# frankaging/Multimodal-Transformer

Hardware: AMD Instinct MI355X
Metric: windows/sec fwd+bwd (higher is better)
Workload: dtype bf16; 1 GPU; SFT encoder stack T=500 d_model=128 heads=8 N=6 d_ff=128, 32 sequences/GPU; fwd + MSE loss + bwd (input, weight, LayerNorm grads); global_batch=32, seq_len=500, d_model=128, heads=8, layers=6, d_ff=128, parallelism=dp1, dropout=train mode, p=0.10 at the reference's four encoder sites, in-kernel generator, lengths=full

## Files before the change

multimodal_transformer_amd/csrc/api.hip:

```cpp
#include <hip/hip_runtime.h>
#include <stdarg.h>
#include <stdio.h>
#include <string.h>
#include <math.h>
#include <stdlib.h>
#include <mutex>
#include <type_traits>
#include <unordered_set>

#include "../../include/mmt_hip.h"
#include "common.h"
#include "rowgemm.h"
#include "attn_mask.h"
#include "attn.h"
#include "attn_bwd_pair.h"
#include "attn_probs.h"
#ifdef MMT_ABLATIONS
#include "attn_bwd_pair_diag.h"
#include "attn_fwd_diag.h"
#endif
#include "misc_kernels.h"
#include "scan_common.h"
#include "scan.h"
#include "mfn_scan.h"
#include "scan_units.h"
#include "scan256.h"
#include "scan_cluster.h"
#include "scan_stack_plan.h"
#include "scan_stack.h"
#include "scan_fb_plan.h"
#include "scan_fb.h"
#include "convpool.h"
#include "convk.h"
#include "glue.h"
#include "local_attn.h"
#include "ar_combine.h"

static thread_local char g_err[512] = "";
static int fail(int code, const char* fmt, ...) {
    va_list ap; va_start(ap, fmt); vsnprintf(g_err, sizeof(g_err), fmt, ap); va_end(ap);
    return code;
}
#define HIP_TRY(expr) do { hipError_t e_ = (expr); if (e_ != hipSuccess) \
    return fail(MMT_EHIP, "%s failed: %s (%s:%d)", #expr, hipGetErrorString(e_), __FILE__, __LINE__); } while (0)

static int ensure_dynamic_lds(const void* kernel) {
// ... 224 lines not shown
        W.slab_stride = set_bytes / sizeof(float);
        for (int l = 1; l < D.N; ++l) c.take<char>(set_bytes);
    }
    for (int l = 0; l < D.N; ++l) { W.lw[l].maskQ = nullptr; W.lw[l].maskK = nullptr; }
    if (train) {
        const size_t lw = attn_mask_layer_words(D.B * D.h, D.nt);
        uint16_t* mq = c.take<uint16_t>(lw * (size_t)(D.N > 0 ? D.N : 1));
        uint16_t* mk = c.take<uint16_t>(lw * (size_t)(D.N > 0 ? D.N : 1));
        for (int l = 0; l < D.N; ++l) { W.lw[l].maskQ = mq ? mq + lw * l : nullptr; W.lw[l].maskK = mk ? mk + lw * l : nullptr; }
    }
    W.bytes = c.off;
}

template <int EPI, bool LN, bool WIDE = false, bool DEVSEED = false>
static int launch_rowgemm(const RowGemmParams& p, hipStream_t st, int site = S_OTHER) {
    if (EPI == EPI_LNBWD && !WIDE && p.no_gs) return launch_rowgemm<EPI_LNBWD, false, true>(p, st, site);
    if (EPI == EPI_PLAIN && !DEVSEED && p.seedword) return launch_rowgemm<EPI_PLAIN, LN, WIDE, true>(p, st, site);
    if (!WIDE && (p.no_gs || p.kchunk)) return fail(MMT_EINVAL, "K-chunked staging / single-tile column sums exist for the LayerNorm-backward kernel only");
    const size_t lds = rowgemm_lds_bytes(EPI, LN, p.KP, p.NP, p.kchunk, p.no_gs != 0);
    if (lds > 160 * 1024) return fail(MMT_EUNSUPPORTED, "row GEMM tile needs %zu B of LDS (K=%d, N=%d)", lds, p.K, p.N);
    if (WIDE && p.kchunk && (!p.a_bf16 || (p.kchunk & (p.kchunk - 1)) || p.kchunk < 64 || p.A_out))
        return fail(MMT_EINVAL, "K-chunked staging needs a bf16 A matrix, a power-of-two chunk >= 64 and no A copy");
    ProfScope prof(site, st);
    return launch("rowgemm_kernel", rowgemm_kernel<EPI, LN, WIDE, DEVSEED>, dim3((p.M + MMT_ROWS - 1) / MMT_ROWS), dim3(MMT_RTHREADS), lds, st, p);
}

static int launch_rowgemm_fixed(void (*kernel)(RowGemmParams), const RowGemmParams& p, size_t lds, hipStream_t st, int site, const char* name) {
    ProfScope prof(site, st);
    return launch(name, kernel, dim3((p.M + MMT_ROWS - 1) / MMT_ROWS), dim3(MMT_RTHREADS), lds, st, p);
}

static int chain_extra_kp(const RowChain3&) { return 0; }
static int chain_extra_kp(const RowChain4& ch) { return ch.d.KP; }

template <typename CH>
static int launch_rowchain(void (*kernel)(CH), CH& ch, bool lnbwd, int site, const char* name, hipStream_t st, int lnb_np = 0, int shape = 0) {
    const int kmax = std::max(std::max(staged_kp(ch.a.KP, ch.a.kchunk), ch.b.KP), std::max(ch.c.KP, chain_extra_kp(ch)));
    const ChainGeom g = chain_geom(kmax, lnbwd ? (lnb_np ? lnb_np : ch.b.NP) : 0, ch.a.no_gs || ch.b.no_gs || ch.c.no_gs, ch.ldx, ch.lda2);
    ch.lda_max = g.lda_max; ch.ldf = g.ldf;
    const bool with_g = g.with_g;
    const size_t lds = g.lds;
    if (lds > 160 * 1024) return fail(MMT_EUNSUPPORTED, "fused row chain needs %zu B of LDS", lds);
    if (shape == 128) {
        const bool ok = ch.ldf == MMT_FIX128_LDF && ch.lda2 == MMT_FIX128_LDA2 && (ch.lda_max == MMT_FIX128_LDA_FWD || ch.lda_max == MMT_FIX128_LDA_BND)
                        && with_g == lnbwd && ch.ldx == (lnbwd ? 0 : 132);
        if (!ok) return fail(MMT_EHIP, "internal: LDS geometry of %s (%d, %d, %d, %d) is not the fixed instance's", name, ch.lda_max, ch.ldf, ch.ldx, ch.lda2);
    }
    if (shape == 256) {
        const bool ok = ch.lda2 == MMT_FIX256_LDA2 && !with_g &&
                        (lnbwd ? (ch.ldf == MMT_FIX256_LDF_BWD && ch.ldx == 0 && (ch.lda_max == MMT_FIX256_LDA || ch.lda_max == MMT_FIX256_LDA_BND))
                               : (ch.ldf == MMT_FIX256_LDF_FWD && ch.ldx == MMT_FIX256_LDX && ch.lda_max == MMT_FIX256_LDA));
        if (!ok) return fail(MMT_EHIP, "internal: LDS geometry of %s (%d, %d, %d, %d) is not the fixed instance's", name, ch.lda_max, ch.ldf, ch.ldx, ch.lda2);
    }
    ProfScope prof(site, st);
    return launch(name, kernel, dim3((ch.a.M + MMT_ROWS - 1) / MMT_ROWS), dim3(MMT_RTHREADS), lds, st, ch);
}

static int chain_shape(int d, int f, int h, const LayerLayout& L) {
    static const bool off = getenv("MMT_NO_FIXED_SHAPES") != nullptr;
    if (off) return 0;
    if (d == 128 && L.DP == 128 && f == 128 && L.FP == 128 && L.HDP == 128 && L.NQ == 384 && h == 8 && L.DKP == 16) return 128;
    if (d == 256 && L.DP == 256 && f == 128 && L.FP == 128 && L.HDP == 256 && L.NQ == 768 && h == 8 && L.DKP == 32) return 256;
    return 0;
}
static RowGemmParams rg_zero() { RowGemmParams p; memset(&p, 0, sizeof(p)); p.mask_scale = 1.0f; return p; }

static DropCfg no_drop() { return make_drop(0.f, 0, 0); }
#define MMT_ATTN_DROP_BITS 12
static DropCfg stream_drop(float p, uint64_t seed, uint32_t stream, bool devseed, int bits = 16, uint32_t first = 0) {
    DropCfg c = make_drop(p, seed, stream, bits);
    if (devseed) { c.s0 = stream - first; c.s1 = 0; }
    return c;
}
static int launch_seed_advance(uint64_t* state, uint64_t* block, uint32_t first, int n, hipStream_t st) {
    if (n + 1 > MMT_SEED_BLOCK_WORDS) return fail(MMT_EUNSUPPORTED, "%d dropout streams do not fit the seed block", n);
    return launch("seed_advance_kernel", seed_advance_kernel, dim3(1), dim3(128), 0, st, state, block, first, n);
}

static int fill_mask_gen(MaskGenParams& P, uint16_t* mq, uint16_t* mk, const EncDims& D, int nlayers, float p, uint64_t seed,
                         const uint64_t* seedword = nullptr) {
    if (nlayers > 16) return fail(MMT_EUNSUPPORTED, "mask generator: %d layers > 16", nlayers);
    memset(&P, 0, sizeof(P));
    P.lq = mq; P.lk = mk; P.nbh = D.B * D.h; P.nt = D.nt; P.nlayers = nlayers;
    P.layer_words = attn_mask_layer_words(P.nbh, P.nt);
    P.seedword = seedword;
    for (int l = 0; l < nlayers; ++l) { const DropCfg c = stream_drop(p, seed, 4 * l + 0, seedword != nullptr, MMT_ATTN_DROP_BITS); P.thr16 = c.thr16; P.s0[l] = c.s0; P.s1[l] = c.s1; }
    return MMT_OK;
}
// ... 83 lines not shown
extern "C" size_t mmt_encoder_workspace_bytes(int B, int T, int d, int h, int f, int n_layers) {
    EncDims D;
    if (make_dims(D, B, T, d, h, f, n_layers) != MMT_OK) return 0;
    EncWs W; carve_encoder(W, D, nullptr, true);
    return W.bytes;
}
extern "C" size_t mmt_encoder_workspace_bytes_eval(int B, int T, int d, int h, int f, int n_layers) {
    EncDims D;
    if (make_dims(D, B, T, d, h, f, n_layers) != MMT_OK) return 0;
    EncWs W; carve_encoder(W, D, nullptr, false);
    return W.bytes;
}

static const float LOG2E = 1.4426950408889634f;

static int encoder_forward_impl(const float* x, const float* mask, const float* params, float* y,
                                void* workspace, size_t workspace_bytes,
                                int B, int T, int d, int h, int f, int n_layers, float eps,
                                float dropout_p, uint64_t seed, uint64_t* seed_state, mmt_stream_t stream) {
    EncDims D;
    int rc = make_dims(D, B, T, d, h, f, n_layers);
    if (rc) return rc;
    if (!x || !mask || !params || !y || !workspace) return fail(MMT_EINVAL, "null pointer argument");
    if ((rc = check_drop(dropout_p, D))) return rc;
    EncWs W; carve_encoder(W, D, workspace, dropout_p > 0.f);
    if ((rc = check_workspace(workspace_bytes, W.bytes))) return rc;
    hipStream_t st = static_cast<hipStream_t>(stream);
    const LayerLayout& L = D.L;
    const bool devseed = seed_state != nullptr && dropout_p > 0.f;
    const uint64_t* seedword = devseed ? W.seedword : nullptr;
    if (devseed && (rc = launch_seed_advance(seed_state, W.seedword, 0, 4 * D.N + 4, st))) return rc;
    auto mkdrop = [&](int stream_id) { return stream_drop(dropout_p, seed, (uint32_t)stream_id, devseed, (stream_id & 3) == 0 ? MMT_ATTN_DROP_BITS : 16); };

    if (D.N > 0 && dropout_p > 0.f) {
        MaskGenParams P;
        if ((rc = fill_mask_gen(P, W.lw[0].maskQ, W.lw[0].maskK, D, D.N, dropout_p, seed, seedword))) return rc;
        const size_t blocks = (size_t)P.nbh * P.nt * P.nt;
        const int gen_blocks = (int)((blocks + 255) / 256), prep_blocks = std::min(grid_for(L.pstride() + L.qstride()), 64);
        ProfScope prof(S_MASK_GEN, st);
        LAUNCH(encoder_prep_maskgen_kernel, dim3((unsigned)(gen_blocks + prep_blocks), D.N), dim3(256), 0, st,
                           params, W.wprep, W.bprep, L, gen_blocks, P);
    } else if (D.N > 0) {
        ProfScope prof(S_PREP, st);
        LAUNCH(encoder_prep_kernel, dim3(grid_for(L.pstride() + L.qstride()), D.N), dim3(256), 0, st,
                           params, W.wprep, W.bprep, L);
    }
    const float* xin = x;
    const int shape = chain_shape(d, f, h, L);
    static const bool fuse_next_qkv = getenv("MMT_NO_CHAIN4") == nullptr;
    for (int l = 0; l < D.N; ++l) {
        const LayerWs& w = W.lw[l];
        const float* P = params + (size_t)l * L.stride();
        const bf16* wp = W.wprep + (size_t)l * L.pstride();
        const float* bp = W.bprep + (size_t)l * L.qstride();
        auto qkv_params = [&](int ll, const float* src) {
            const LayerWs& wl = W.lw[ll];
            const float* Pl = params + (size_t)ll * L.stride();
            RowGemmParams p = rg_zero();
            p.M = D.M; p.K = d; p.KP = L.DP; p.N = 3 * L.HD; p.NP = L.NQ;
            p.A = src; p.lda = d; p.A_out = wl.xn1; p.lda_out = L.DP;
            p.ln_a = Pl + L.oln(0); p.ln_b = Pl + L.oln(1); p.eps = eps; p.stats = wl.stats1;
            p.W = W.wprep + (size_t)ll * L.pstride() + L.pWqkv(); p.bias = W.bprep + (size_t)ll * L.qstride() + L.qbqkv();
            p.fragR[0] = wl.QR; p.fragR[1] = wl.KR; p.fragR[2] = wl.VR;
            p.T = T; p.Tp = D.Tp; p.h = h; p.DKP = L.DKP; p.nwhich = 3;
            p.rowmask = mask; p.qscale = LOG2E / sqrtf((float)L.dk); p.scale_first = 1;
            return p;
        };
        if (l == 0) {
            RowGemmParams p = qkv_params(0, xin);
            if (shape == 128) rc = launch_rowgemm_fixed(encoder_ln1_qkv128_kernel, p, rowgemm_lds_bytes(EPI_FRAG, true, 128, 384), st, S_LN1_QKV, "encoder_ln1_qkv128_kernel");
            else rc = launch_rowgemm<EPI_FRAG, true>(p, st, S_LN1_QKV);
            if (rc) return rc;
        }
        if ((rc = launch_attn_fwd(L.DKP, w.QR, w.KR, w.VR, w.ctx, w.lse, D, st, mkdrop(4 * l + 0), w.maskQ))) return rc;
        {
            RowChain3 ch; memset(&ch, 0, sizeof(ch));
            {   RowGemmParams& p = ch.a; p = rg_zero();
                p.M = D.M; p.K = L.HDP; p.KP = L.HDP; p.N = d; p.NP = L.DP;
                p.A = w.ctx; p.a_bf16 = 1; p.lda = L.HDP;
                p.W = wp + L.pWo(); p.bias = bp + L.qbo();
                p.residual = xin; p.ldr = d; p.out_f32 = w.x1; p.ldo = d;
                p.drop = mkdrop(4 * l + 1); p.seedword = seedword; }
            {   RowGemmParams& p = ch.b; p = rg_zero();
                p.M = D.M; p.K = d; p.KP = L.DP; p.N = f; p.NP = L.FP;
                p.A_out = w.xn2; p.lda_out = L.DP;
                p.ln_a = P + L.oln(2); p.ln_b = P + L.oln(3); p.eps = eps; p.stats = w.stats2;
                p.W = wp + L.pW1(); p.bias = bp + L.qb1(); p.act = 1;
                p.out_bf16 = w.hid; p.ldo16 = L.FP; p.n_store16 = L.FP;
                p.drop = mkdrop(4 * l + 2); p.seedword = seedword; }
            {   RowGemmParams& p = ch.c; p = rg_zero();
                p.M = D.M; p.K = L.FP; p.KP = L.FP; p.N = d; p.NP = L.DP;
                p.W = wp + L.pW2(); p.bias = bp + L.qb2();
                p.out_f32 = w.xout; p.ldo = d;
                p.drop = mkdrop(4 * l + 3); p.seedword = seedword; }
            ch.ldx = L.DP + 4; ch.lda2 = L.FP + 8;
            if (l + 1 < D.N && fuse_next_qkv) {
                RowChain4 c4; memset(&c4, 0, sizeof(c4));
                c4.a = ch.a; c4.b = ch.b; c4.c = ch.c; c4.ldx = ch.ldx; c4.lda2 = ch.lda2;
                c4.d = qkv_params(l + 1, nullptr);
                if ((rc = with_shape(devseed, shape, [&](auto ds, auto sh) {
                        return launch_rowchain(encoder_post_attn_fwd4_kernel<CT(ds), CT(sh)>, c4, false, S_CHAIN4_FWD, "encoder_post_attn_fwd4_kernel", st, 0, shape);
                    }))) return rc;
            } else {
                if (l + 1 == D.N) {
                    const float* Pf = params + (size_t)D.N * L.stride();
                    ch.ln.a = Pf; ch.ln.b = Pf + d; ch.ln.eps = eps; ch.ln.y = y; ch.ln.stats = W.statsf; ch.ln.d = d;
                }
                if ((rc = with_shape(devseed, shape, [&](auto ds, auto sh) {
                        return launch_rowchain(encoder_post_attn_fwd_kernel<CT(ds), CT(sh)>, ch, false, S_OUTPROJ, "encoder_post_attn_fwd_kernel", st, 0, shape);
                    }))) return rc;
                if (l + 1 < D.N) {
                    RowGemmParams p = qkv_params(l + 1, w.xout);
                    if ((rc = launch_rowgemm<EPI_FRAG, true>(p, st, S_LN1_QKV))) return rc;
                }
            }
        }
        xin = w.xout;
    }
    if (D.N == 0) {
        const float* Pf = params;
        ProfScope prof(S_LN_FWD, st);
        LAUNCH(layernorm_fwd_kernel, dim3(D.G), dim3(MMT_THREADS), 0, st, xin, Pf, Pf + d, eps, y, W.statsf, D.M, d);
    }
    return MMT_OK;
}

extern "C" int mmt_encoder_forward(const float* x, const float* mask, const float* params, float* y,
                                   void* workspace, size_t workspace_bytes,
                                   int B, int T, int d, int h, int f, int n_layers, float eps,
                                   float dropout_p, uint64_t seed, mmt_stream_t stream) {
    return encoder_forward_impl(x, mask, params, y, workspace, workspace_bytes, B, T, d, h, f, n_layers, eps, dropout_p, seed, nullptr, stream);
}
// ... 1144 lines not shown
```

multimodal_transformer_amd/csrc/attn_mask.h:

```cpp
#pragma once
#include "common.h"

#define MMT_MASK_BLOCK_WORDS 32

__device__ __forceinline__ void attn_keep_block(const DropCfg& dc, uint32_t blk, uint32_t (&W)[32]) {
    const uint32_t thr = dc.thr16;
    const int b0 = thr ? __builtin_ctz(thr) : 16;
#pragma unroll
    for (int key = 0; key < 32; ++key) W[key] = 0;
    uint32_t x = drop_lin(dc.s0, blk * 512u) + (uint32_t)b0 * MMT_DROP_C1;
#pragma unroll 1
    for (int b = b0; b < 16; ++b) {
        if ((thr >> b) & 1u) {
#pragma unroll
            for (int key = 0; key < 32; ++key) W[key] |= drop_fin(x + (uint32_t)(16 * key) * MMT_DROP_C1, dc.s1);
        } else {
#pragma unroll
            for (int key = 0; key < 32; ++key) W[key] &= drop_fin(x + (uint32_t)(16 * key) * MMT_DROP_C1, dc.s1);
        }
        x += MMT_DROP_C1;
    }
#pragma unroll
    for (int key = 0; key < 32; ++key) W[key] = ~W[key];
}

__device__ __forceinline__ void transpose32(uint32_t (&A)[32]) {
#pragma unroll
    for (int s = 0; s < 5; ++s) {
        const int j = 16 >> s;
        const uint32_t m = (s == 0) ? 0x0000FFFFu : (s == 1) ? 0x00FF00FFu : (s == 2) ? 0x0F0F0F0Fu : (s == 3) ? 0x33333333u : 0x55555555u;
#pragma unroll
        for (int k = 0; k < 32; ++k) {
            if (k & j) continue;
            const uint32_t t = ((A[k] >> j) ^ A[k + j]) & m;
            A[k + j] ^= t;
            A[k] ^= t << j;
        }
    }
}

__device__ __forceinline__ uint32_t lane_word(uint32_t x, int hh) {
    uint32_t y = (x >> (4 * hh)) & 0x0F0F0F0Fu;
    y = (y | (y >> 4)) & 0x00FF00FFu;
    return (y | (y >> 8)) & 0x0000FFFFu;
}

struct MaskGenParams {
    uint16_t* lq; uint16_t* lk;
    size_t layer_words;
    int nbh, nt, nlayers;
    uint32_t thr16;
    uint32_t s0[16], s1[16];
    const uint64_t* seedword;
};

#define MMT_MASK_LDS_ROW 72
__device__ __forceinline__ void park_lane_block(uint16_t* row, const uint32_t (&rows)[32]) {
#pragma unroll
    for (int c = 0; c < 8; ++c) {
        u32x4_t v;
#pragma unroll
        for (int e = 0; e < 4; ++e) {
            const int l0 = 8 * (c & 3) + 2 * e, hh = c >> 2;
            v[e] = lane_word(rows[l0], hh) | (lane_word(rows[l0 + 1], hh) << 16);
        }
        *reinterpret_cast<u32x4_t*>(row + 8 * c) = v;
    }
}

__device__ __forceinline__ void attn_mask_gen_block(const MaskGenParams& P, int layer, int bx) {
    __shared__ __attribute__((aligned(16))) uint16_t patch[4][64 * MMT_MASK_LDS_ROW];
    const int lane = threadIdx.x & 63, wave = threadIdx.x >> 6;
    const size_t g0 = (size_t)bx * 256 + wave * 64;
    const size_t per_bh = (size_t)P.nt * P.nt, total = (size_t)P.nbh * per_bh;
    if (g0 >= total) return;
    const size_t g = g0 + lane;
    const bool live = g < total;
    const size_t gc = live ? g : total - 1;
    const int bh = (int)(gc / per_bh);
    const int rem = (int)(gc - (size_t)bh * per_bh), qt = rem / P.nt, kt = rem - qt * P.nt;
    DropCfg base; base.thr16 = P.thr16; base.scale = 1.f; base.s0 = P.s0[layer]; base.s1 = P.s1[layer];
    const DropCfg dc = drop_substream(drop_resolve(base, P.seedword), (uint32_t)bh);
    uint32_t W[32];
    attn_keep_block(dc, (uint32_t)(qt * P.nt + kt), W);
    uint16_t* const mine = patch[wave] + lane * MMT_MASK_LDS_ROW;
    const int fp = lane & 7;
    const uint16_t* const from = patch[wave] + (lane >> 3) * MMT_MASK_LDS_ROW + 8 * fp;
    park_lane_block(mine, W);
    {
        size_t gb = g0 + (lane >> 3);
        int bb = (int)((gb < total ? gb : total - 1) / per_bh);
        int rb = (int)((gb < total ? gb : total - 1) - (size_t)bb * per_bh), qb = rb / P.nt, kb = rb - qb * P.nt;
        uint16_t* const lk = P.lk + (size_t)layer * P.layer_words;
#pragma unroll
        for (int i = 0; i < 8; ++i) {
            const u32x4_t v = *reinterpret_cast<const u32x4_t*>(from + 8 * i * MMT_MASK_LDS_ROW);
            if (gb < total) *reinterpret_cast<u32x4_t*>(lk + ((size_t)bb * per_bh + (size_t)kb * P.nt + qb) * 64 + 8 * fp) = v;
            gb += 8; kb += 8;
            while (kb >= P.nt) { kb -= P.nt; if (++qb == P.nt) { qb = 0; ++bb; } }
        }
    }
    transpose32(W);
    park_lane_block(mine, W);
    {
        uint16_t* const lq = P.lq + (size_t)layer * P.layer_words + g0 * 64;
#pragma unroll
        for (int i = 0; i < 8; ++i) {
            const u32x4_t v = *reinterpret_cast<const u32x4_t*>(from + 8 * i * MMT_MASK_LDS_ROW);
            if (g0 + 8 * i + (lane >> 3) < total) *reinterpret_cast<u32x4_t*>(lq + (size_t)i * 512 + lane * 8) = v;
        }
    }
}

__global__ __launch_bounds__(256, 4) void attn_mask_gen_kernel(const MaskGenParams P) { attn_mask_gen_block(P, blockIdx.y, blockIdx.x); }

__host__ inline size_t attn_mask_layer_words(int nbh, int nt) { return (size_t)nbh * nt * nt * 64; }

template <int I> struct IdxC { static constexpr int value = I; };
template <int B, int E, class F> __device__ __forceinline__ void static_for(F&& f) {
    if constexpr (B < E) { f(IdxC<B>{}); static_for<B + 1, E>(f); }
}
template <int I> __device__ __forceinline__ uint32_t keep_bits(uint32_t w) {
    uint32_t m;
    asm("v_bfe_i32 %0, %1, %2, 1" : "=v"(m) : "v"(w), "n"(I));
    return m;
}
template <int I> __device__ __forceinline__ float keep_and(float v, uint32_t w) {
    return __builtin_bit_cast(float, __builtin_bit_cast(uint32_t, v) & keep_bits<I>(w));
}

__global__ void attn_mask_expand_kernel(DropCfg base, int nbh, int nt, uint8_t* __restrict__ keep) {
    const size_t g = (size_t)blockIdx.x * blockDim.x + threadIdx.x;
    const size_t per_bh = (size_t)nt * nt;
    const int bh = (int)(g / per_bh);
    if (bh >= nbh) return;
    const int rem = (int)(g - (size_t)bh * per_bh), qt = rem / nt, kt = rem - qt * nt;
    const DropCfg dc = drop_substream(base, (uint32_t)bh);
    uint32_t W[32];
    attn_keep_block(dc, (uint32_t)(qt * nt + kt), W);
    const size_t Tp = (size_t)nt * 32;
#pragma unroll
    for (int key = 0; key < 32; ++key)
#pragma unroll 1
        for (int q = 0; q < 32; ++q)
            keep[((size_t)bh * Tp + qt * 32 + q) * Tp + kt * 32 + key] = (W[key] >> q) & 1u;
}
```

multimodal_transformer_amd/csrc/misc_kernels.h:

```cpp
#pragma once
#include "common.h"

struct LayerLayout {
    int d, f, h, dk, DKP, HD, HDP, DP, FP, NQ;
    __host__ __device__ size_t oW(int i) const { return (size_t)i * ((size_t)d * d + d); }
    __host__ __device__ size_t ob(int i) const { return oW(i) + (size_t)d * d; }
    __host__ __device__ size_t oW1() const { return oW(4); }
    __host__ __device__ size_t ob1() const { return oW1() + (size_t)f * d; }
    __host__ __device__ size_t oW2() const { return ob1() + f; }
    __host__ __device__ size_t ob2() const { return oW2() + (size_t)d * f; }
    __host__ __device__ size_t oln(int i) const { return ob2() + d + (size_t)i * d; }
    __host__ __device__ size_t stride() const { return oln(4); }
    __host__ __device__ size_t pWqkv() const { return 0; }
    __host__ __device__ size_t pWqkvT() const { return pWqkv() + (size_t)NQ * DP; }
    __host__ __device__ size_t pWo() const { return pWqkvT() + (size_t)DP * NQ; }
    __host__ __device__ size_t pWoT() const { return pWo() + (size_t)DP * HDP; }
    __host__ __device__ size_t pW1() const { return pWoT() + (size_t)HDP * DP; }
    __host__ __device__ size_t pW1T() const { return pW1() + (size_t)FP * DP; }
    __host__ __device__ size_t pW2() const { return pW1T() + (size_t)DP * FP; }
    __host__ __device__ size_t pW2T() const { return pW2() + (size_t)DP * FP; }
    __host__ __device__ size_t pstride() const { return pW2T() + (size_t)FP * DP; }
    __host__ __device__ size_t qbqkv() const { return 0; }
    __host__ __device__ size_t qbo() const { return NQ; }
    __host__ __device__ size_t qb1() const { return (size_t)NQ + DP; }
// ... 51 lines not shown
            const int n = (int)(i / L.HDP), c = (int)(i % L.HDP);
            if (n < d) { const int s = unpad_head(c, L); if (s >= 0) v = P[L.oW(3) + (size_t)n * d + s]; }
        } else if (idx < L.pW1()) {
            const size_t i = idx - L.pWoT();
            const int c = (int)(i / L.DP), n = (int)(i % L.DP);
            if (n < d) { const int s = unpad_head(c, L); if (s >= 0) v = P[L.oW(3) + (size_t)n * d + s]; }
        } else if (idx < L.pW1T()) {
            const size_t i = idx - L.pW1();
            const int n = (int)(i / L.DP), k = (int)(i % L.DP);
            if (n < f && k < d) v = P[L.oW1() + (size_t)n * d + k];
        } else if (idx < L.pW2()) {
            const size_t i = idx - L.pW1T();
            const int k = (int)(i / L.FP), n = (int)(i % L.FP);
            if (n < f && k < d) v = P[L.oW1() + (size_t)n * d + k];
        } else if (idx < L.pW2T()) {
            const size_t i = idx - L.pW2();
            const int n = (int)(i / L.FP), k = (int)(i % L.FP);
            if (n < d && k < f) v = P[L.oW2() + (size_t)n * f + k];
        } else {
            const size_t i = idx - L.pW2T();
            const int k = (int)(i / L.DP), n = (int)(i % L.DP);
            if (n < d && k < f) v = P[L.oW2() + (size_t)n * f + k];
        }
        W[idx] = (bf16)v;
    }
}
__global__ void encoder_prep_kernel(const float* __restrict__ params, bf16* __restrict__ wprep,
                                    float* __restrict__ bprep, LayerLayout L) {
    encoder_prep_block(params, wprep, bprep, L, blockIdx.y, blockIdx.x, gridDim.x);
}
__global__ __launch_bounds__(256, 4) void encoder_prep_maskgen_kernel(const float* __restrict__ params, bf16* __restrict__ wprep,
                                                                      float* __restrict__ bprep, LayerLayout L, int gen_blocks,
                                                                      const MaskGenParams P) {
    if ((int)blockIdx.x >= gen_blocks) { encoder_prep_block(params, wprep, bprep, L, blockIdx.y, blockIdx.x - gen_blocks, gridDim.x - gen_blocks); return; }
    attn_mask_gen_block(P, blockIdx.y, blockIdx.x);
}

__global__ void pad_cast_kernel(const float* __restrict__ src, bf16* __restrict__ dst, int N, int K, int NP, int KP,
                                int transpose_src) {
    const size_t total = (size_t)NP * KP;
    for (size_t idx = (size_t)blockIdx.x * blockDim.x + threadIdx.x; idx < total; idx += (size_t)gridDim.x * blockDim.x) {
        const int n = (int)(idx / KP), k = (int)(idx % KP);
        float v = 0.f;
        if (n < N && k < K) v = transpose_src ? src[(size_t)k * N + n] : src[(size_t)n * K + k];
        dst[idx] = (bf16)v;
    }
}

__global__ void pad_f32_kernel(const float* __restrict__ src, float* __restrict__ dst, int n, int np) {
    const int i = blockIdx.x * blockDim.x + threadIdx.x;
    if (i < np) dst[i] = (i < n && src) ? src[i] : 0.f;
}

__global__ void grad_prep_kernel(const float* __restrict__ dy, const float* __restrict__ y, const float* __restrict__ rowscale,
                                 int act, bf16* __restrict__ g, int M, int N, int NP, float gscale) {
    const size_t total = (size_t)M * (NP >> 2);
    for (size_t idx = (size_t)blockIdx.x * blockDim.x + threadIdx.x; idx < total; idx += (size_t)gridDim.x * blockDim.x) {
        const int m = (int)(idx / (NP >> 2)), n = (int)(idx % (NP >> 2)) * 4;
        bf16x4 o;
#pragma unroll
        for (int i = 0; i < 4; ++i) {
            float v = 0.f;
            if (n + i < N) {
                v = dy[(size_t)m * N + n + i];
                if (rowscale) v *= rowscale[m];
                if (act == 1) { v = (y[(size_t)m * N + n + i] > 0.f) ? v * gscale : 0.f; }
                else if (act == 2) { const float yy = y[(size_t)m * N + n + i]; v *= 1.f - yy * yy; }
                else if (act == 3) { const float yy = y[(size_t)m * N + n + i]; v *= yy * (1.f - yy); }
// ... 382 lines not shown
```

multimodal_transformer_amd/csrc/rowgemm.h:

```cpp
#pragma once
#include "common.h"

enum { EPI_PLAIN = 0, EPI_FRAG = 1, EPI_LNBWD = 2 };

#ifndef MMT_ROWS
#define MMT_ROWS 32
#endif
#ifndef MMT_RTHREADS
#define MMT_RTHREADS 512
#endif
static_assert(MMT_ROWS == 16 || MMT_ROWS == 32, "row tile must be 16 or 32 windows");
static_assert(MMT_RTHREADS == 256 || MMT_RTHREADS == 512, "row kernels run 4 or 8 waves");
static_assert(MMT_RTHREADS / MMT_ROWS == 8 || MMT_RTHREADS / MMT_ROWS == 16, "8 or 16 threads per row");
#define MMT_RNW (MMT_RTHREADS / 64)
#define MMT_RTPR (MMT_RTHREADS / MMT_ROWS)
#define MMT_RSTEP (MMT_RTHREADS / 32)
#define MMT_RIT (MMT_ROWS / MMT_RSTEP)
#define MMT_WCOLS (128 / MMT_RNW)
#define MMT_WNT (MMT_WCOLS / 16)
struct RowGemmParams {
    int M, K, KP, N, NP;
    const void* A; int a_bf16; int lda;
    bf16* A_out; int lda_out;
    DropCfg a_drop;
    const float* ln_a; const float* ln_b; float eps; float* stats;
    const bf16* W; const float* bias;
    int act;
    const bf16* relu_mask; int ldm; float mask_scale;
    DropCfg drop;
    const float* residual; int ldr;
    const float* rowscale;
    float* out_f32; int ldo;
    bf16* out_bf16; int ldo16; int n_store16;
    bf16* fragR[3];
// ... 579 lines not shown
                        }
                    }
                }
                float* dst = p.colpart + (size_t)blockIdx.x * 2 * NP;
                dst[c] = sb; dst[NP + c] = sa;
            }
        }
        __syncthreads();
    }
}

__device__ __forceinline__ void warm_weights(const bf16* W, int NP, int KP) {
    if ((blockIdx.x & (MMT_ROWS == 16 ? 7 : 3)) != 0) return;
    const int lines = (NP * KP) >> 6;
    unsigned acc = 0;
    for (int l = threadIdx.x; l < lines; l += MMT_RTHREADS) acc |= *reinterpret_cast<const unsigned*>(W + (size_t)l * 64);
    asm volatile("" :: "v"(acc));
}

template <int EPI, bool LNPRO, bool WIDE = false, bool DEVSEED = false>
__global__ __launch_bounds__(MMT_RTHREADS, (MMT_ROWS == 16 || MMT_RTHREADS == 512) ? 4 : 2) void rowgemm_kernel(const RowGemmParams p) {
    extern __shared__ __attribute__((aligned(16))) char smem[];
    RowSmem sm;
    sm.As = reinterpret_cast<bf16*>(smem);
    sm.Fs = reinterpret_cast<float*>(smem + (size_t)MMT_ROWS * ((p.kchunk > 0 && p.kchunk < p.KP ? p.kchunk : p.KP) + 8) * 2);
    sm.ldf = rowgemm_fw(EPI, LNPRO, p.KP, p.NP) + 4;
    sm.Gs = sm.Fs + (size_t)MMT_ROWS * sm.ldf;
    sm.Xs = nullptr; sm.A2 = nullptr; sm.ldx = 0; sm.lda2 = 0;
    rowgemm_stage<EPI, LNPRO, ASRC_GLOBAL, 0, DEVSEED, WIDE>(p, sm);
}

struct LnOut { const float* a; const float* b; float eps; float* y; float* stats; int d; };
struct RowChain3 { RowGemmParams a, b, c; int lda_max, ldf, ldx, lda2; LnOut ln; };
struct RowChain4 { RowGemmParams a, b, c, d; int lda_max, ldf, ldx, lda2; };

template <typename CH>
__host__ __device__ inline size_t rowchain_lds_bytes(const CH& ch, bool with_g) {
    return (size_t)MMT_ROWS * ch.lda_max * 2 + (size_t)MMT_ROWS * ch.ldf * 4 * (with_g ? 2 : 1) + (size_t)MMT_ROWS * ch.ldx * 4 + (size_t)MMT_ROWS * ch.lda2 * 2;
}
template <typename CH>
__device__ __forceinline__ RowSmem rowchain_carve(char* smem, const CH& ch, bool with_g) {
    RowSmem sm;
    sm.As = reinterpret_cast<bf16*>(smem);
    sm.Fs = reinterpret_cast<float*>(smem + (size_t)MMT_ROWS * ch.lda_max * 2);
    sm.ldf = ch.ldf;
    sm.Gs = sm.Fs + (size_t)MMT_ROWS * ch.ldf;
    sm.Xs = sm.Fs + (size_t)MMT_ROWS * ch.ldf * (with_g ? 2 : 1);
    sm.ldx = ch.ldx;
    sm.A2 = reinterpret_cast<bf16*>(sm.Xs + (size_t)MMT_ROWS * ch.ldx);
    sm.lda2 = ch.lda2;
    return sm;
}

__device__ __forceinline__ void ln_tile_out(const float* Xs, int ldx, const LnOut& lo, int M) {
    constexpr int TPR = MMT_RTPR;
    const int row = threadIdx.x / TPR, j = threadIdx.x % TPR, m = blockIdx.x * MMT_ROWS + row, K = lo.d;
    const float* xr = Xs + row * ldx;
    float s = 0.f;
    for (int c = j * 4; c < K; c += 4 * TPR) { f32x4 v = *reinterpret_cast<const f32x4*>(xr + c); s += (v[0] + v[1]) + (v[2] + v[3]); }
    s += __shfl_xor(s, 1); s += __shfl_xor(s, 2); s += __shfl_xor(s, 4);
    if (TPR == 16) s += __shfl_xor(s, 8);
    const float mean = s / (float)K;
    float q = 0.f;
    for (int c = j * 4; c < K; c += 4 * TPR) {
        f32x4 v = *reinterpret_cast<const f32x4*>(xr + c);
#pragma unroll
        for (int i = 0; i < 4; ++i) { const float t = v[i] - mean; q += t * t; }
// ... 77 lines not shown
    p.ldr = N_; p.ldo = N_; p.ldo16 = N_; p.n_store16 = N_; p.ldm = N_;
    p.ldx = N_; p.lddres = N_; p.d_real = N_; p.next_lda = N_ + 8; p.ldctx = N_;
    return p;
}
template <int LDA_MAX, int LDF, bool WITH_G, int LDX, int LDA2>
__device__ __forceinline__ RowSmem carve_fixed(char* smem) {
    RowSmem sm;
    sm.As = reinterpret_cast<bf16*>(smem);
    sm.Fs = reinterpret_cast<float*>(smem + (size_t)MMT_ROWS * LDA_MAX * 2);
    sm.ldf = LDF;
    sm.Gs = sm.Fs + (size_t)MMT_ROWS * LDF;
    sm.Xs = sm.Fs + (size_t)MMT_ROWS * LDF * (WITH_G ? 2 : 1);
    sm.ldx = LDX;
    sm.A2 = reinterpret_cast<bf16*>(sm.Xs + (size_t)MMT_ROWS * LDX);
    sm.lda2 = LDA2;
    return sm;
}
#define MMT_FIX128_LDF 132
#define MMT_FIX128_LDA2 136
#define MMT_FIX128_LDA_FWD 136
#define MMT_FIX128_LDA_BND 392
__device__ __forceinline__ RowGemmParams qkv128(RowGemmParams p) { p = shape_pin<128, 384>(p); p.lda_out = 128; p.h = 8; p.DKP = 16; return p; }
__device__ __forceinline__ RowGemmParams dO128(RowGemmParams p) { p = shape_pin<128, 128>(p); p.h = 8; p.DKP = 16; return p; }
#define MMT_FIX256_LDA 264
#define MMT_FIX256_LDA_BND 520
#define MMT_FIX256_LDF_FWD 132
#define MMT_FIX256_LDF_BWD 260
#define MMT_FIX256_LDX 260
#define MMT_FIX256_LDA2 136
__device__ __forceinline__ RowGemmParams qkv256(RowGemmParams p) { p = shape_pin<256, 768>(p); p.lda_out = 256; p.h = 8; p.DKP = 32; return p; }
__device__ __forceinline__ RowGemmParams dO256(RowGemmParams p) { p = shape_pin<256, 256>(p); p.h = 8; p.DKP = 32; return p; }
__device__ __forceinline__ RowGemmParams lnbwd256(RowGemmParams p) { p.no_gs = 1; return p; }

template <bool DEVSEED, int SHAPE = 0>
__global__ __launch_bounds__(MMT_RTHREADS, (MMT_ROWS == 16 || MMT_RTHREADS == 512) ? 4 : 2) void encoder_post_attn_fwd4_kernel(const RowChain4 ch) {
    extern __shared__ __attribute__((aligned(16))) char smem[];
    warm_weights(ch.b.W, ch.b.NP, ch.b.KP); warm_weights(ch.c.W, ch.c.NP, ch.c.KP);
    warm_weights(ch.d.W, ch.d.NP, ch.d.KP);
    if (SHAPE == 128) {
        const RowSmem sm = carve_fixed<MMT_FIX128_LDA_FWD, MMT_FIX128_LDF, false, 132, MMT_FIX128_LDA2>(smem);
        rowgemm_stage<EPI_PLAIN, false, ASRC_GLOBAL, KEEP_X, DEVSEED>(shape_pin<128, 128>(role_plain(ch.a)), sm);
        rowgemm_stage<EPI_PLAIN, true, ASRC_X, KEEP_A2, DEVSEED>(shape_pin<128, 128>(role_ffn1(ch.b)), sm);
        rowgemm_stage<EPI_PLAIN, false, ASRC_A2, RES_X | KEEP_X, DEVSEED>(shape_pin<128, 128>(role_plain(ch.c)), sm);
        rowgemm_stage<EPI_FRAG, true, ASRC_X, 0, false>(qkv128(role_qkv(ch.d)), sm);
        return;
    }
    if (SHAPE == 256) {
        const RowSmem sm = carve_fixed<MMT_FIX256_LDA, MMT_FIX256_LDF_FWD, false, MMT_FIX256_LDX, MMT_FIX256_LDA2>(smem);
        rowgemm_stage<EPI_PLAIN, false, ASRC_GLOBAL, KEEP_X, DEVSEED>(shape_pin<256, 256>(role_plain(ch.a)), sm);
        rowgemm_stage<EPI_PLAIN, true, ASRC_X, KEEP_A2, DEVSEED>(shape_pin<256, 128>(role_ffn1(ch.b)), sm);
        rowgemm_stage<EPI_PLAIN, false, ASRC_A2, RES_X | KEEP_X, DEVSEED>(shape_pin<128, 256>(role_plain(ch.c)), sm);
        rowgemm_stage<EPI_FRAG, true, ASRC_X, 0, false>(qkv256(role_qkv(ch.d)), sm);
        return;
    }
    const RowSmem sm = rowchain_carve(smem, ch, false);
    rowgemm_stage<EPI_PLAIN, false, ASRC_GLOBAL, KEEP_X, DEVSEED>(role_plain(ch.a), sm);
    rowgemm_stage<EPI_PLAIN, true, ASRC_X, KEEP_A2, DEVSEED>(role_ffn1(ch.b), sm);
    rowgemm_stage<EPI_PLAIN, false, ASRC_A2, RES_X | KEEP_X, DEVSEED>(role_plain(ch.c), sm);
    rowgemm_stage<EPI_FRAG, true, ASRC_X, 0, false>(role_qkv(ch.d), sm);
}

__global__ __launch_bounds__(MMT_RTHREADS, (MMT_ROWS == 16 || MMT_RTHREADS == 512) ? 4 : 2) void encoder_ln1_qkv128_kernel(const RowGemmParams p) {
    extern __shared__ __attribute__((aligned(16))) char smem[];
    const RowSmem sm = carve_fixed<MMT_FIX128_LDA_FWD, MMT_FIX128_LDF, false, 0, 0>(smem);
    RowGemmParams q = qkv128(role_qkv(p));
    q.lda = 128;
    rowgemm_stage<EPI_FRAG, true, ASRC_GLOBAL, 0, false>(q, sm);
}
template <bool DEVSEED>
// ... 62 lines not shown
```

Measured before the change: 20.02 million windows/s.

## Generate next layer's dropout masks inside the fused post-attention chain kernel

Instead of generating every layer's attention dropout keep-masks upfront in the prep kernel, only layer 0's masks are built there. Each later layer's masks are produced by extra workgroups appended to the previous layer's post-attention chain kernel, running at low priority alongside the row GEMMs to use idle CU capacity. The chain kernel's launch-bounds occupancy is raised for the 128 shape, and the keep-block generator is split into smaller groups of keys to lower register pressure. Mask addressing now uses shuffles instead of recomputed divisions. Risks include register and occupancy pressure on the GEMM path and contention that could slow the chain stages.

```diff
diff --git a/multimodal_transformer_amd/csrc/api.hip b/multimodal_transformer_amd/csrc/api.hip
--- a/multimodal_transformer_amd/csrc/api.hip
+++ b/multimodal_transformer_amd/csrc/api.hip
@@ -10,8 +10,8 @@
 
 #include "../../include/mmt_hip.h"
 #include "common.h"
+#include "attn_mask.h"
 #include "rowgemm.h"
-#include "attn_mask.h"
 #include "attn.h"
 #include "attn_bwd_pair.h"
 #include "attn_probs.h"
@@ -302,6 +302,16 @@
 
 static int chain_extra_kp(const RowChain3&) { return 0; }
 static int chain_extra_kp(const RowChain4& ch) { return ch.d.KP; }
+static int chain_ride_wgs(const RowChain3&) { return 0; }
+static int chain_ride_wgs(const RowChain4& ch) { return ch.ride.gen_wgs; }
+
+static int mask_ride_waves(int shape, size_t chain_lds) {
+    static const bool off = getenv("MMT_NO_MASK_RIDE") != nullptr;
+    if (off || shape != 128 || MMT_RTHREADS != 512) return 0;
+    const size_t wgs_per_cu = (size_t)MMT_RIDE_OCC * 4 / (MMT_RTHREADS / 64);
+    if (wgs_per_cu < 3 || wgs_per_cu * chain_lds > 160 * 1024) return 0;
+    return (int)std::min<size_t>(MMT_RIDE_WAVES, chain_lds / (MMT_MASK_PATCH_WORDS * sizeof(uint16_t)));
+}
 
 template <typename CH>
 static int launch_rowchain(void (*kernel)(CH), CH& ch, bool lnbwd, int site, const char* name, hipStream_t st, int lnb_np = 0, int shape = 0) {
@@ -322,8 +332,10 @@
                                : (ch.ldf == MMT_FIX256_LDF_FWD && ch.ldx == MMT_FIX256_LDX && ch.lda_max == MMT_FIX256_LDA));
         if (!ok) return fail(MMT_EHIP, "internal: LDS geometry of %s (%d, %d, %d, %d) is not the fixed instance's", name, ch.lda_max, ch.ldf, ch.ldx, ch.lda2);
     }
+    if (chain_ride_wgs(ch) && (shape != 128 || lnbwd || mask_ride_waves(shape, lds) <= 0))
+        return fail(MMT_EHIP, "internal: %s cannot carry mask generator workgroups", name);
     ProfScope prof(site, st);
-    return launch(name, kernel, dim3((ch.a.M + MMT_ROWS - 1) / MMT_ROWS), dim3(MMT_RTHREADS), lds, st, ch);
+    return launch(name, kernel, dim3((ch.a.M + MMT_ROWS - 1) / MMT_ROWS + chain_ride_wgs(ch)), dim3(MMT_RTHREADS), lds, st, ch);
 }
 
 static int chain_shape(int d, int f, int h, const LayerLayout& L) {
@@ -473,9 +485,15 @@
     if (devseed && (rc = launch_seed_advance(seed_state, W.seedword, 0, 4 * D.N + 4, st))) return rc;
     auto mkdrop = [&](int stream_id) { return stream_drop(dropout_p, seed, (uint32_t)stream_id, devseed, (stream_id & 3) == 0 ? MMT_ATTN_DROP_BITS : 16); };
 
+    const int shape = chain_shape(d, f, h, L);
+    static const bool fuse_next_qkv = getenv("MMT_NO_CHAIN4") == nullptr;
+    const int ride_waves = (dropout_p > 0.f && fuse_next_qkv)
+        ? mask_ride_waves(shape, chain_geom(std::max(std::max(L.HDP, L.DP), L.FP), 0, false, L.DP + 4, L.FP + 8).lds) : 0;
+    MaskGenParams MG;
     if (D.N > 0 && dropout_p > 0.f) {
-        MaskGenParams P;
-        if ((rc = fill_mask_gen(P, W.lw[0].maskQ, W.lw[0].maskK, D, D.N, dropout_p, seed, seedword))) return rc;
+        if ((rc = fill_mask_gen(MG, W.lw[0].maskQ, W.lw[0].maskK, D, D.N, dropout_p, seed, seedword))) return rc;
+        MaskGenParams P = MG;
+        if (ride_waves) P.nlayers = 1;
         const size_t blocks = (size_t)P.nbh * P.nt * P.nt;
         const int gen_blocks = (int)((blocks + 255) / 256), prep_blocks = std::min(grid_for(L.pstride() + L.qstride()), 64);
         ProfScope prof(S_MASK_GEN, st);
@@ -487,8 +505,6 @@
                            params, W.wprep, W.bprep, L);
     }
     const float* xin = x;
-    const int shape = chain_shape(d, f, h, L);
-    static const bool fuse_next_qkv = getenv("MMT_NO_CHAIN4") == nullptr;
     for (int l = 0; l < D.N; ++l) {
         const LayerWs& w = W.lw[l];
         const float* P = params + (size_t)l * L.stride();
@@ -539,6 +555,14 @@
                 RowChain4 c4; memset(&c4, 0, sizeof(c4));
                 c4.a = ch.a; c4.b = ch.b; c4.c = ch.c; c4.ldx = ch.ldx; c4.lda2 = ch.lda2;
                 c4.d = qkv_params(l + 1, nullptr);
+                c4.ride.chain_wgs = (D.M + MMT_ROWS - 1) / MMT_ROWS;
+                if (ride_waves) {
+                    MaskGenLayer& g = c4.ride.g;
+                    g.lq = W.lw[l + 1].maskQ; g.lk = W.lw[l + 1].maskK; g.nbh = MG.nbh; g.nt = MG.nt;
+                    g.thr16 = MG.thr16; g.s0 = MG.s0[l + 1]; g.s1 = MG.s1[l + 1]; g.seedword = MG.seedword;
+                    const size_t blocks = (size_t)g.nbh * g.nt * g.nt, per_wg = (size_t)64 * ride_waves;
+                    c4.ride.gen_waves = ride_waves; c4.ride.gen_wgs = (int)((blocks + per_wg - 1) / per_wg);
+                }
                 if ((rc = with_shape(devseed, shape, [&](auto ds, auto sh) {
                         return launch_rowchain(encoder_post_attn_fwd4_kernel<CT(ds), CT(sh)>, c4, false, S_CHAIN4_FWD, "encoder_post_attn_fwd4_kernel", st, 0, shape);
                     }))) return rc;
diff --git a/multimodal_transformer_amd/csrc/attn_mask.h b/multimodal_transformer_amd/csrc/attn_mask.h
--- a/multimodal_transformer_amd/csrc/attn_mask.h
+++ b/multimodal_transformer_amd/csrc/attn_mask.h
@@ -3,25 +3,32 @@
 
 #define MMT_MASK_BLOCK_WORDS 32
 
+template <int CHAINS = 32>
 __device__ __forceinline__ void attn_keep_block(const DropCfg& dc, uint32_t blk, uint32_t (&W)[32]) {
+    static_assert(CHAINS > 0 && 32 % CHAINS == 0, "the keys of a block are drawn in equal groups");
     const uint32_t thr = dc.thr16;
     const int b0 = thr ? __builtin_ctz(thr) : 16;
+    const uint32_t x0 = drop_lin(dc.s0, blk * 512u) + (uint32_t)b0 * MMT_DROP_C1;
 #pragma unroll
-    for (int key = 0; key < 32; ++key) W[key] = 0;
-    uint32_t x = drop_lin(dc.s0, blk * 512u) + (uint32_t)b0 * MMT_DROP_C1;
+    for (int k0 = 0; k0 < 32; k0 += CHAINS) {
+        uint32_t D[CHAINS];
+#pragma unroll
+        for (int i = 0; i < CHAINS; ++i) D[i] = 0;
+        uint32_t x = x0;
 #pragma unroll 1
-    for (int b = b0; b < 16; ++b) {
-        if ((thr >> b) & 1u) {
+        for (int b = b0; b < 16; ++b) {
+            if ((thr >> b) & 1u) {
 #pragma unroll
-            for (int key = 0; key < 32; ++key) W[key] |= drop_fin(x + (uint32_t)(16 * key) * MMT_DROP_C1, dc.s1);
-        } else {
+                for (int i = 0; i < CHAINS; ++i) D[i] |= drop_fin(x + (uint32_t)(16 * (k0 + i)) * MMT_DROP_C1, dc.s1);
+            } else {
 #pragma unroll
-            for (int key = 0; key < 32; ++key) W[key] &= drop_fin(x + (uint32_t)(16 * key) * MMT_DROP_C1, dc.s1);
+                for (int i = 0; i < CHAINS; ++i) D[i] &= drop_fin(x + (uint32_t)(16 * (k0 + i)) * MMT_DROP_C1, dc.s1);
+            }
+            x += MMT_DROP_C1;
         }
-        x += MMT_DROP_C1;
+#pragma unroll
+        for (int i = 0; i < CHAINS; ++i) W[k0 + i] = ~D[i];
     }
-#pragma unroll
-    for (int key = 0; key < 32; ++key) W[key] = ~W[key];
 }
 
 __device__ __forceinline__ void transpose32(uint32_t (&A)[32]) {
@@ -53,6 +60,18 @@
     uint32_t s0[16], s1[16];
     const uint64_t* seedword;
 };
+struct MaskGenLayer {
+    uint16_t* lq; uint16_t* lk;
+    int nbh, nt;
+    uint32_t thr16, s0, s1;
+    const uint64_t* seedword;
+};
+__device__ __forceinline__ MaskGenLayer mask_gen_layer(const MaskGenParams& P, int layer) {
+    MaskGenLayer G;
+    G.lq = P.lq + (size_t)layer * P.layer_words; G.lk = P.lk + (size_t)layer * P.layer_words;
+    G.nbh = P.nbh; G.nt = P.nt; G.thr16 = P.thr16; G.s0 = P.s0[layer]; G.s1 = P.s1[layer]; G.seedword = P.seedword;
+    return G;
+}
 
 #define MMT_MASK_LDS_ROW 72
 __device__ __forceinline__ void park_lane_block(uint16_t* row, const uint32_t (&rows)[32]) {
@@ -68,10 +87,14 @@
     }
 }
 
-__device__ __forceinline__ void attn_mask_gen_block(const MaskGenParams& P, int layer, int bx) {
-    __shared__ __attribute__((aligned(16))) uint16_t patch[4][64 * MMT_MASK_LDS_ROW];
-    const int lane = threadIdx.x & 63, wave = threadIdx.x >> 6;
-    const size_t g0 = (size_t)bx * 256 + wave * 64;
+#define MMT_MASK_PATCH_WORDS (64 * MMT_MASK_LDS_ROW)
+#define MMT_MASK_GEN_WAVES 4
+template <int CHAINS = 32>
+__device__ __forceinline__ void attn_mask_gen_block(const MaskGenLayer& P, uint16_t* patch, size_t first, int gen_waves) {
+    const int lane = threadIdx.x & 63, wave = __builtin_amdgcn_readfirstlane(threadIdx.x >> 6);
+    if (wave >= gen_waves) return;
+    patch += wave * MMT_MASK_PATCH_WORDS;
+    const size_t g0 = first + wave * 64;
     const size_t per_bh = (size_t)P.nt * P.nt, total = (size_t)P.nbh * per_bh;
     if (g0 >= total) return;
     const size_t g = g0 + lane;
@@ -79,31 +102,32 @@
     const size_t gc = live ? g : total - 1;
     const int bh = (int)(gc / per_bh);
     const int rem = (int)(gc - (size_t)bh * per_bh), qt = rem / P.nt, kt = rem - qt * P.nt;
-    DropCfg base; base.thr16 = P.thr16; base.scale = 1.f; base.s0 = P.s0[layer]; base.s1 = P.s1[layer];
+    DropCfg base; base.thr16 = P.thr16; base.scale = 1.f; base.s0 = P.s0; base.s1 = P.s1;
     const DropCfg dc = drop_substream(drop_resolve(base, P.seedword), (uint32_t)bh);
     uint32_t W[32];
-    attn_keep_block(dc, (uint32_t)(qt * P.nt + kt), W);
-    uint16_t* const mine = patch[wave] + lane * MMT_MASK_LDS_ROW;
+    attn_keep_block<CHAINS>(dc, (uint32_t)(qt * P.nt + kt), W);
+    uint16_t* const mine = patch + lane * MMT_MASK_LDS_ROW;
     const int fp = lane & 7;
-    const uint16_t* const from = patch[wave] + (lane >> 3) * MMT_MASK_LDS_ROW + 8 * fp;
+    const uint16_t* from;
+    auto flush_from = [&] { int l = lane; asm volatile("" : "+v"(l)); return patch + (l >> 3) * MMT_MASK_LDS_ROW + 8 * (l & 7); };
     park_lane_block(mine, W);
+    from = flush_from();
     {
         size_t gb = g0 + (lane >> 3);
-        int bb = (int)((gb < total ? gb : total - 1) / per_bh);
-        int rb = (int)((gb < total ? gb : total - 1) - (size_t)bb * per_bh), qb = rb / P.nt, kb = rb - qb * P.nt;
-        uint16_t* const lk = P.lk + (size_t)layer * P.layer_words;
+        int bb = __shfl(bh, lane >> 3), qb = __shfl(qt, lane >> 3), kb = __shfl(kt, lane >> 3);
 #pragma unroll
         for (int i = 0; i < 8; ++i) {
             const u32x4_t v = *reinterpret_cast<const u32x4_t*>(from + 8 * i * MMT_MASK_LDS_ROW);
-            if (gb < total) *reinterpret_cast<u32x4_t*>(lk + ((size_t)bb * per_bh + (size_t)kb * P.nt + qb) * 64 + 8 * fp) = v;
+            if (gb < total) *reinterpret_cast<u32x4_t*>(P.lk + ((size_t)bb * per_bh + (size_t)kb * P.nt + qb) * 64 + 8 * fp) = v;
             gb += 8; kb += 8;
             while (kb >= P.nt) { kb -= P.nt; if (++qb == P.nt) { qb = 0; ++bb; } }
         }
     }
     transpose32(W);
     park_lane_block(mine, W);
+    from = flush_from();
     {
-        uint16_t* const lq = P.lq + (size_t)layer * P.layer_words + g0 * 64;
+        uint16_t* const lq = P.lq + g0 * 64;
 #pragma unroll
         for (int i = 0; i < 8; ++i) {
             const u32x4_t v = *reinterpret_cast<const u32x4_t*>(from + 8 * i * MMT_MASK_LDS_ROW);
@@ -112,7 +136,10 @@
     }
 }
 
-__global__ __launch_bounds__(256, 4) void attn_mask_gen_kernel(const MaskGenParams P) { attn_mask_gen_block(P, blockIdx.y, blockIdx.x); }
+__global__ __launch_bounds__(256, 4) void attn_mask_gen_kernel(const MaskGenParams P) {
+    __shared__ __attribute__((aligned(16))) uint16_t patch[MMT_MASK_GEN_WAVES * MMT_MASK_PATCH_WORDS];
+    attn_mask_gen_block(mask_gen_layer(P, blockIdx.y), patch, (size_t)blockIdx.x * (64 * MMT_MASK_GEN_WAVES), MMT_MASK_GEN_WAVES);
+}
 
 __host__ inline size_t attn_mask_layer_words(int nbh, int nt) { return (size_t)nbh * nt * nt * 64; }
 
diff --git a/multimodal_transformer_amd/csrc/misc_kernels.h b/multimodal_transformer_amd/csrc/misc_kernels.h
--- a/multimodal_transformer_amd/csrc/misc_kernels.h
+++ b/multimodal_transformer_amd/csrc/misc_kernels.h
@@ -107,8 +107,10 @@
 __global__ __launch_bounds__(256, 4) void encoder_prep_maskgen_kernel(const float* __restrict__ params, bf16* __restrict__ wprep,
                                                                       float* __restrict__ bprep, LayerLayout L, int gen_blocks,
                                                                       const MaskGenParams P) {
+    __shared__ __attribute__((aligned(16))) uint16_t patch[MMT_MASK_GEN_WAVES * MMT_MASK_PATCH_WORDS];
     if ((int)blockIdx.x >= gen_blocks) { encoder_prep_block(params, wprep, bprep, L, blockIdx.y, blockIdx.x - gen_blocks, gridDim.x - gen_blocks); return; }
-    attn_mask_gen_block(P, blockIdx.y, blockIdx.x);
+    if ((int)blockIdx.y >= P.nlayers) return;
+    attn_mask_gen_block(mask_gen_layer(P, blockIdx.y), patch, (size_t)blockIdx.x * (64 * MMT_MASK_GEN_WAVES), MMT_MASK_GEN_WAVES);
 }
 
 __global__ void pad_cast_kernel(const float* __restrict__ src, bf16* __restrict__ dst, int N, int K, int NP, int KP,
diff --git a/multimodal_transformer_amd/csrc/rowgemm.h b/multimodal_transformer_amd/csrc/rowgemm.h
--- a/multimodal_transformer_amd/csrc/rowgemm.h
+++ b/multimodal_transformer_amd/csrc/rowgemm.h
@@ -1,5 +1,6 @@
 #pragma once
 #include "common.h"
+#include "attn_mask.h"
 
 enum { EPI_PLAIN = 0, EPI_FRAG = 1, EPI_LNBWD = 2 };
 
@@ -645,7 +646,8 @@
 
 struct LnOut { const float* a; const float* b; float eps; float* y; float* stats; int d; };
 struct RowChain3 { RowGemmParams a, b, c; int lda_max, ldf, ldx, lda2; LnOut ln; };
-struct RowChain4 { RowGemmParams a, b, c, d; int lda_max, ldf, ldx, lda2; };
+struct MaskRide { MaskGenLayer g; int chain_wgs, gen_wgs, gen_waves; };
+struct RowChain4 { RowGemmParams a, b, c, d; int lda_max, ldf, ldx, lda2; MaskRide ride; };
 
 template <typename CH>
 __host__ __device__ inline size_t rowchain_lds_bytes(const CH& ch, bool with_g) {
@@ -789,9 +791,19 @@
 __device__ __forceinline__ RowGemmParams dO256(RowGemmParams p) { p = shape_pin<256, 256>(p); p.h = 8; p.DKP = 32; return p; }
 __device__ __forceinline__ RowGemmParams lnbwd256(RowGemmParams p) { p.no_gs = 1; return p; }
 
+#define MMT_RIDE_WAVES 4
+#define MMT_RIDE_CHAINS 16
+#define MMT_RIDE_OCC 6
 template <bool DEVSEED, int SHAPE = 0>
-__global__ __launch_bounds__(MMT_RTHREADS, (MMT_ROWS == 16 || MMT_RTHREADS == 512) ? 4 : 2) void encoder_post_attn_fwd4_kernel(const RowChain4 ch) {
+__global__ __launch_bounds__(MMT_RTHREADS, (MMT_ROWS == 16 || MMT_RTHREADS == 512) ? ((SHAPE == 128 && MMT_RTHREADS == 512) ? MMT_RIDE_OCC : 4) : 2)
+void encoder_post_attn_fwd4_kernel(const RowChain4 ch) {
     extern __shared__ __attribute__((aligned(16))) char smem[];
+    if (SHAPE == 128 && (int)blockIdx.x >= ch.ride.chain_wgs) {
+        __builtin_amdgcn_s_setprio(0);
+        attn_mask_gen_block<MMT_RIDE_CHAINS>(ch.ride.g, reinterpret_cast<uint16_t*>(smem),
+                                             (size_t)((int)blockIdx.x - ch.ride.chain_wgs) * (64 * ch.ride.gen_waves), ch.ride.gen_waves);
+        return;
+    }
     warm_weights(ch.b.W, ch.b.NP, ch.b.KP); warm_weights(ch.c.W, ch.c.NP, ch.c.KP);
     warm_weights(ch.d.W, ch.d.NP, ch.d.KP);
     if (SHAPE == 128) {
```

Measured after the change: 20.76 million windows/s (median of 6 runs). 3.7% higher.
